# paulmillr/noble-curves

Hardware: NVIDIA H100
Metric: BLS12-381 G1 MSM points/sec at 2^20 scalars (higher is better)
Workload: dtype u32-limb integer (381-bit Fp, Montgomery)

## Files before the change

noble-curves_b200/csrc/capi.cu:

```cuda
#include <dlfcn.h>
#include <thread>
#include <nccl.h>

#include "context.h"
#include "curve_consts.cuh"
#include "field.cuh"

namespace nmsm {

Context g_ctx;
std::mutex g_mu;
DistState g_dist;

struct NcclApi {
  void* handle = nullptr;
  ncclResult_t (*GetUniqueId)(ncclUniqueId*) = nullptr;
  ncclResult_t (*CommInitRank)(ncclComm_t*, int, ncclUniqueId, int) = nullptr;
  ncclResult_t (*CommDestroy)(ncclComm_t) = nullptr;
  ncclResult_t (*Send)(const void*, size_t, ncclDataType_t, int, ncclComm_t, cudaStream_t) = nullptr;
  ncclResult_t (*Recv)(void*, size_t, ncclDataType_t, int, ncclComm_t, cudaStream_t) = nullptr;
  ncclResult_t (*AllGather)(const void*, void*, size_t, ncclDataType_t, ncclComm_t, cudaStream_t) = nullptr;
  ncclResult_t (*GroupStart)() = nullptr;
  ncclResult_t (*GroupEnd)() = nullptr;
  const char* (*GetErrorString)(ncclResult_t) = nullptr;
// ... 222 lines not shown
  CK(cudaMemcpyAsync(d_h + D.world, &mine, sizeof(mine), cudaMemcpyHostToDevice, st));
  if (int r = nccl_all_gather(d_h + D.world, d_h, sizeof(mine), st)) { cudaFree(d_h); return r; }
  std::vector<cudaIpcMemHandle_t> all(D.world);
  CK(cudaMemcpyAsync(all.data(), d_h, sizeof(mine) * D.world, cudaMemcpyDeviceToHost, st));
  CK(cudaStreamSynchronize(st));
  cudaFree(d_h);
  uint32_t ok = 1;
  for (int r = 0; r < D.world; r++) {
    if (r == D.rank) continue;
    cudaError_t e = cudaIpcOpenMemHandle(&D.mapped[slot][r], all[r], cudaIpcMemLazyEnablePeerAccess);
    if (e != cudaSuccess) {
      (void)cudaGetLastError();
      D.mapped[slot][r] = nullptr;
      ok = 0;
    }
  }
  uint32_t* d_ok = nullptr;
  CK(cudaMalloc((void**)&d_ok, 4 * (D.world + 1)));
  CK(cudaMemcpyAsync(d_ok + D.world, &ok, 4, cudaMemcpyHostToDevice, st));
  if (int r = nccl_all_gather(d_ok + D.world, d_ok, 4, st)) { cudaFree(d_ok); return r; }
  std::vector<uint32_t> oks(D.world);
  CK(cudaMemcpyAsync(oks.data(), d_ok, 4 * D.world, cudaMemcpyDeviceToHost, st));
  CK(cudaStreamSynchronize(st));
  cudaFree(d_ok);
  for (uint32_t v : oks) ok &= v;
  if (!ok) {
    for (int r = 0; r < D.world; r++)
      if (D.mapped[slot][r]) {
        cudaIpcCloseMemHandle(D.mapped[slot][r]);
        D.mapped[slot][r] = nullptr;
      }
    D.p2p = false;
    return NMSM_OK;
  }
  D.mapped_local[slot] = local_base;
  return NMSM_OK;
}

}

using namespace nmsm;

#define ENGINE(curve)                                      \
  const EngineVTable* E = engine_for(curve);               \
  if (!E) return fail(NMSM_ERR_ARG, "unknown curve id")
#define SLOT0_FREE()                                                                                         \
  if (g_ctx.slot[0].pend.active)                                                                             \
  return fail(NMSM_ERR_ARG, "slot 0 holds an MSM that has not been collected: collect it before a synchronous call")

extern "C" {

int nmsm_init(int device) {
  std::lock_guard<std::mutex> lk(g_mu);
  Context& C = g_ctx;
  if (C.ready && C.device == device) return NMSM_OK;
  if (C.ready) return fail(NMSM_ERR_ARG, "nmsm_init: context already bound to another device");
  setenv("CUDA_DEVICE_MAX_CONNECTIONS", "32", 0);
  int count = 0;
  cudaError_t e = cudaGetDeviceCount(&count);
  if (e != cudaSuccess || count == 0)
    return fail(NMSM_ERR_CUDA, std::string("no CUDA device available (there is no CPU fallback): ") +
                                   cudaGetErrorString(e));
  if (device < 0 || device >= count) return fail(NMSM_ERR_ARG, "nmsm_init: bad device ordinal");
  CK(cudaSetDevice(device));
  cudaDeviceProp prop;
  CK(cudaGetDeviceProperties(&prop, device));
  C.sm_count = prop.multiProcessorCount;
  int prio_lo = 0, prio_hi = 0;
  CK(cudaDeviceGetStreamPriorityRange(&prio_lo, &prio_hi));
  for (Slot& S : C.slot) {
    CK(cudaStreamCreateWithFlags(&S.stream, cudaStreamNonBlocking));
    for (auto& st : S.acc_stream) CK(cudaStreamCreateWithPriority(&st, cudaStreamNonBlocking, prio_lo));
    for (auto& st : S.tail_stream) CK(cudaStreamCreateWithPriority(&st, cudaStreamNonBlocking, prio_hi));
    CK(cudaStreamCreateWithPriority(&S.horner_stream, cudaStreamNonBlocking, prio_hi));
    CK(cudaStreamCreateWithFlags(&S.prep_stream, cudaStreamNonBlocking));
    CK(cudaEventCreateWithFlags(&S.ev_start, cudaEventDisableTiming));
    CK(cudaEventCreateWithFlags(&S.ev_prep, cudaEventDisableTiming));
    CK(cudaMallocHost((void**)&S.h_result, 1024));
    for (auto& ev : S.ev) CK(cudaEventCreate(&ev));
    CK(cudaEventCreateWithFlags(&S.done, cudaEventDisableTiming));
    CK(cudaEventCreateWithFlags(&S.ev_fork, cudaEventDisableTiming));
    CK(cudaEventCreateWithFlags(&S.ev_horner, cudaEventDisableTiming));
    for (auto& ev : S.ev_acc) CK(cudaEventCreateWithFlags(&ev, cudaEventDisableTiming));
    for (auto& ev : S.ev_tail) CK(cudaEventCreateWithFlags(&ev, cudaEventDisableTiming));
    CK(cudaEventCreate(&S.ev_t0));
    CK(cudaEventCreate(&S.ev_t1));
    if (getenv("NMSM_TRACE")) {
      C.trace = true;
      CK(cudaEventCreate(&S.tr_fork));
      for (auto& ev : S.tr_acc) CK(cudaEventCreate(&ev));
      for (auto& ev : S.tr_tail) CK(cudaEventCreate(&ev));
      for (auto& ev : S.tr_h) CK(cudaEventCreate(&ev));
    }
    CK(cudaStreamCreateWithPriority(&S.comm_stream, cudaStreamNonBlocking, prio_hi));
    CK(cudaEventCreateWithFlags(&S.ev_gather, cudaEventDisableTiming));
    for (auto& ev : S.ev_fin) CK(cudaEventCreateWithFlags(&ev, cudaEventDisableTiming));
    for (auto& ev : S.ev_xchg) CK(cudaEventCreateWithFlags(&ev, cudaEventDisableTiming));
    CK(cudaMallocHost((void**)&S.h_gather, 64 * 1024));
  }
  C.device = device;
  C.ready = true;
  return NMSM_OK;
}

void nmsm_shutdown(void) {
  std::lock_guard<std::mutex> lk(g_mu);
  Context& C = g_ctx;
  if (!C.ready) return;
  if (g_dist.ready) {
    for (Slot& S : C.slot) cudaStreamSynchronize(S.comm_stream);
    for (int sl = 0; sl < NUM_SLOTS; sl++)
      for (int r = 0; r < MAX_PEERS; r++)
        if (g_dist.mapped[sl][r]) cudaIpcCloseMemHandle(g_dist.mapped[sl][r]);
    g_nccl.CommDestroy((ncclComm_t)g_dist.comm);
    g_dist = DistState();
  }
  for (Slot& S : C.slot) {
    cudaStreamSynchronize(S.stream);
    cudaStreamSynchronize(S.comm_stream);
    for (auto st : S.acc_stream) cudaStreamSynchronize(st);
    for (auto st : S.tail_stream) cudaStreamSynchronize(st);
    cudaStreamSynchronize(S.horner_stream);
    cudaStreamSynchronize(S.prep_stream);
    for (Buf* b : {&S.in_pts, &S.in_scalars, &S.aff, &S.counts, &S.offsets, &S.cursor, &S.sorted, &S.buckets, &S.heads,
                   &S.tails, &S.chunk_out, &S.window_out, &S.tile_sums, &S.blk, &S.tiles, &S.result, &S.mul_out, &S.hacc,
                   &S.recv, &S.gsend, &S.grecv})
      b->release();
    for (auto& ev : S.ev_fin) cudaEventDestroy(ev);
    for (auto& ev : S.ev_xchg) cudaEventDestroy(ev);
    cudaEventDestroy(S.ev_gather);
    cudaFreeHost(S.h_gather);
    cudaStreamDestroy(S.comm_stream);
    for (auto& ev : S.ev) cudaEventDestroy(ev);
    for (auto& ev : S.ev_acc) cudaEventDestroy(ev);
    for (auto& ev : S.ev_tail) cudaEventDestroy(ev);
    for (cudaEvent_t ev : {S.done, S.ev_fork, S.ev_horner, S.ev_t0, S.ev_t1}) cudaEventDestroy(ev);
    cudaFreeHost(S.h_result);
    for (auto st : S.acc_stream) cudaStreamDestroy(st);
    for (auto st : S.tail_stream) cudaStreamDestroy(st);
    cudaStreamDestroy(S.horner_stream);
    cudaStreamDestroy(S.prep_stream);
    cudaEventDestroy(S.ev_start);
    cudaEventDestroy(S.ev_prep);
    cudaStreamDestroy(S.stream);
    S.pend = Pending();
  }
  h2d_release();
  C.ed_scratch.release();
  cudaFree(C.secp256k1_g_table);
  C.secp256k1_g_table = nullptr;
  cudaFree(C.p256_g_table);
  C.p256_g_table = nullptr;
  cudaFree(C.ed25519_b_table);
  C.ed25519_b_table = nullptr;
  for (Buf* b : {&C.ntt_data, &C.ntt_work, &C.ntt_tmp, &C.ntt_roots, &C.ntt_aux}) b->release();
  C.ntt_key_field = -1;
  C.ntt_key_bits = -1;
  C.ready = false;
  C.device = -1;
}

const char* nmsm_last_error(void) {
  static thread_local std::string copy;
  std::lock_guard<std::mutex> lk(g_mu);
  copy = g_ctx.last_error;
  return copy.c_str();
}
long long nmsm_last_error_index(void) {
  std::lock_guard<std::mutex> lk(g_mu);
  return g_ctx.last_error_index;
}

int nmsm_point_bytes(int curve) {
  ENGINE(curve);
  return E->point_bytes;
}
int nmsm_acc_bytes(int curve) {
  ENGINE(curve);
  return E->acc_bytes;
}

int nmsm_msm(int curve, const uint8_t* pts, const uint8_t* scalars, uint64_t n, uint8_t* out_xy, int* out_is_inf) {
  std::lock_guard<std::mutex> lk(g_mu);
  if (int r = ensure_init()) return r;
  g_ctx.cur = 0;
  SLOT0_FREE();
  if (!out_xy || !out_is_inf || (n && (!pts || !scalars))) return fail(NMSM_ERR_ARG, "null pointer");
  ENGINE(curve);
  return E->msm_host(pts, scalars, n, out_xy, out_is_inf);
}

int nmsm_msm_device(int curve, const void* d_pts, const void* d_scalars, uint64_t n, uint8_t* out_xy,
                    int* out_is_inf) {
  std::lock_guard<std::mutex> lk(g_mu);
  if (int r = ensure_init()) return r;
  g_ctx.cur = 0;
  SLOT0_FREE();
  if (!out_xy || !out_is_inf || (n && (!d_pts || !d_scalars))) return fail(NMSM_ERR_ARG, "null pointer");
  ENGINE(curve);
  return E->msm_device((const uint32_t*)d_pts, (const uint32_t*)d_scalars, n, nullptr, out_xy, out_is_inf);
}

int nmsm_msm_partial_device(int curve, const void* d_pts, const void* d_scalars, uint64_t n, void* d_out_acc) {
  std::lock_guard<std::mutex> lk(g_mu);
  if (int r = ensure_init()) return r;
  g_ctx.cur = 0;
  SLOT0_FREE();
  if (!d_out_acc || (n && (!d_pts || !d_scalars))) return fail(NMSM_ERR_ARG, "null pointer");
  ENGINE(curve);
  return E->msm_device((const uint32_t*)d_pts, (const uint32_t*)d_scalars, n, (uint32_t*)d_out_acc, nullptr, nullptr);
}

int nmsm_fold_partials_device(int curve, const void* d_accs, int count, uint8_t* out_xy, int* out_is_inf) {
  std::lock_guard<std::mutex> lk(g_mu);
  if (int r = ensure_init()) return r;
  g_ctx.cur = 0;
  SLOT0_FREE();
// ... 521 lines not shown
```

noble-curves_b200/csrc/context.h:

```cpp
#pragma once
#include <cuda_runtime.h>
#include <stdint.h>
#include <stdio.h>
#include <string.h>

#include <mutex>
#include <string>
#include <vector>

#include "../../include/nmsm.h"

namespace nmsm {
struct MsmPlanLite {
  int c, W, B, G, L, K, chunks, D;
  uint32_t TPW;
};
}

namespace nmsm {

struct Buf {
  void* p = nullptr;
  size_t cap = 0;
  cudaError_t ensure(size_t bytes) {
    if (bytes <= cap) return cudaSuccess;
    if (p) cudaFree(p);
    p = nullptr;
    cap = 0;
    size_t want = bytes + bytes / 8 + 256;
    cudaError_t e = cudaMalloc(&p, want);
    if (e == cudaSuccess) cap = want;
    return e;
  }
  void release() {
    if (p) cudaFree(p);
    p = nullptr;
    cap = 0;
  }
};

struct Pending {
  bool active = false;
  int curve = -1;
  MsmPlanLite plan = {};
  uint64_t n = 0;
  bool partial = false;
  bool empty = false;
  bool sharded = false;
  int gather_words = 0;
  bool profiled = false;
  int groups = 1;
  int launches = 0;
};
static constexpr int MAX_GROUPS = 8;
static constexpr int MAX_WINDOWS = 34;
static constexpr int ACC_STREAMS = 8, TAIL_STREAMS = 4;
struct Slot {
  cudaStream_t stream = nullptr;
  cudaStream_t acc_stream[ACC_STREAMS] = {}, tail_stream[TAIL_STREAMS] = {}, horner_stream = nullptr;
  cudaStream_t prep_stream = nullptr;
  cudaEvent_t ev_start = nullptr, ev_prep = nullptr;
  cudaEvent_t ev_fork = nullptr, ev_acc[MAX_WINDOWS] = {}, ev_tail[MAX_WINDOWS] = {}, ev_horner = nullptr;
  cudaStream_t comm_stream = nullptr;
  cudaEvent_t ev_fin[MAX_WINDOWS] = {}, ev_xchg[MAX_WINDOWS] = {}, ev_gather = nullptr;
  uint32_t* h_gather = nullptr;
  Buf recv, gsend, grecv;
  cudaEvent_t ev_t0 = nullptr, ev_t1 = nullptr;
  cudaEvent_t tr_fork = nullptr, tr_acc[MAX_WINDOWS] = {}, tr_tail[MAX_WINDOWS] = {}, tr_h[MAX_WINDOWS] = {};
  Buf in_pts, in_scalars, aff, counts, offsets, cursor, sorted, buckets, heads, tails, chunk_out, window_out, tile_sums,
      blk, tiles, result, mul_out, hacc;
  uint32_t* h_result = nullptr;
  cudaEvent_t ev[NMSM_TIMING_SLOTS + 2] = {};
  cudaEvent_t done = nullptr;
  float last_ms[NMSM_TIMING_SLOTS] = {};
  nmsm_plan_info last_info = {};
  Pending pend;
};
static constexpr int NUM_SLOTS = NMSM_SLOTS;

struct Context {
  bool ready = false;
  int device = -1;
  int sm_count = 132;
  Slot slot[NUM_SLOTS];
  int cur = 0;
  Buf ed_scratch;
  uint32_t* secp256k1_g_table = nullptr;
  uint32_t* ed25519_b_table = nullptr;
  uint32_t* p256_g_table = nullptr;
  Buf ntt_data, ntt_work, ntt_tmp, ntt_roots, ntt_aux;
  int ntt_key_field = -1, ntt_key_bits = -1;
  uint64_t ntt_key_gen = 0;
  bool profiling = false;
  bool trace = false;
  int forced_c = 0;
  int forced_groups = 0;
  float last_ms[NMSM_TIMING_SLOTS] = {};
  nmsm_plan_info last_info = {};
  std::string last_error;
  long long last_error_index = -1;
};

int h2d_any(void* dst, const void* src, size_t bytes, cudaStream_t stream);
void h2d_release();

struct NcclComm;
static constexpr int MAX_PEERS = 16;
struct PeerPtrs {
  const uint32_t* p[MAX_PEERS];
};
struct DistState {
  bool ready = false;
  int rank = 0, world = 1;
  NcclComm* comm = nullptr;
  bool p2p = false;
  void* mapped[NMSM_SLOTS][MAX_PEERS] = {};
  void* mapped_local[NMSM_SLOTS] = {};
};
int nccl_send(const void* buf, size_t bytes, int peer, cudaStream_t st);
int nccl_recv(void* buf, size_t bytes, int peer, cudaStream_t st);
int nccl_group_start();
int nccl_group_end();
int nccl_all_gather(const void* send, void* recv, size_t bytes_per_rank, cudaStream_t st);
int dist_map_peer_buckets(int slot, void* local_base, cudaStream_t st);
extern DistState g_dist;

struct ShardArgs {
  uint64_t n_total, offset;
};

extern Context g_ctx;
extern std::mutex g_mu;

inline int fail(int code, const std::string& msg, long long idx = -1) {
  g_ctx.last_error = msg;
  g_ctx.last_error_index = idx;
  return code;
}
inline int cuda_fail(cudaError_t e, const char* what) {
  return fail(NMSM_ERR_CUDA, std::string("CUDA error in ") + what + ": " + cudaGetErrorString(e));
}
#define CK(call)                                         \
  do {                                                   \
    cudaError_t e__ = (call);                            \
    if (e__ != cudaSuccess) return cuda_fail(e__, #call); \
  } while (0)

inline int check_offsets(const uint64_t* off, const char* name, uint64_t n) {
  if (off[0] != 0) return fail(NMSM_ERR_ARG, std::string(name) + "[0] must be 0");
  for (uint64_t i = 0; i < n; i++)
    if (off[i + 1] < off[i])
      return fail(NMSM_ERR_ARG, std::string(name) + " must be non-decreasing (index " + std::to_string(i + 1) + ")",
// ... 85 lines not shown
```

noble-curves_b200/csrc/engine.cuh:

```cuda
#pragma once
#include "context.h"
#include "msm.cuh"

namespace nmsm {

inline unsigned int cdiv(uint64_t a, unsigned int b) { return (unsigned int)((a + b - 1) / b); }

#define EV(slot)                                                         \
  do {                                                                   \
    if (g_ctx.profiling) cudaEventRecord(C.ev[slot], C.stream);              \
  } while (0)

template <class Cv>
struct Engine {
  using G = typename Cv::G;

static int run_msm(const uint32_t* d_pts, const uint32_t* d_scalars, uint64_t n, uint32_t* d_out_acc,
                   uint8_t* out_xy, int* out_is_inf, const uint32_t* d_prepared = nullptr, int table_c = 0,
                   uint64_t table_points = 0) {
  if (int r = submit_msm(d_pts, d_scalars, n, d_out_acc, d_prepared, table_c, table_points)) return r;
  return collect_msm(out_xy, out_is_inf);
}

static int reduce2_r(uint64_t chunks) {
  if (chunks <= (uint64_t)REDUCE2_LOGICAL * 4) {
    int r = 1;
    while ((uint64_t)REDUCE2_LOGICAL * r < chunks) r *= 2;
    return r;
  }
  int r = REDUCE2_R;
  while (r < 16 && (chunks + (uint64_t)REDUCE2_LOGICAL * r - 1) / ((uint64_t)REDUCE2_LOGICAL * r) > (uint64_t)REDUCE2_MAX_SPLITS &&
         chunks <= (uint64_t)REDUCE2_LOGICAL * 16 * REDUCE2_MAX_SPLITS)
    r *= 2;
  return r;
}

static constexpr int SHARD_MIN_C = 8;

static int choose_groups(const MsmPlan& plan, uint64_t max_entries) {
  (void)max_entries;
  if (plan.W <= 1) return 1;
  int ng = 1;
  if (g_ctx.forced_groups) ng = g_ctx.forced_groups < plan.W ? g_ctx.forced_groups : plan.W;
  if (g_ctx.profiling) ng = 1;
  return ng;
}

static bool prepare_on_side_stream(uint64_t n, bool prepared) { return !g_ctx.profiling && !prepared && n >= (1u << 14); }

static int stage_host_inputs(Slot& C, const void* pts, const void* scalars, uint64_t n) {
  if (n >= (1ull << 31)) return fail(NMSM_ERR_ARG, "n must be < 2^31");
  CK(C.in_pts.ensure(n * G::IN_WORDS * 4));
  CK(C.in_scalars.ensure(n * SCALAR_WORDS * 4));
  if (int r = h2d_any(C.in_scalars.p, scalars, n * SCALAR_WORDS * 4, C.stream)) return r;
  return h2d_any(C.in_pts.p, pts, n * G::IN_WORDS * 4, prepare_on_side_stream(n, false) ? C.prep_stream : C.stream);
}

static int submit_msm(const uint32_t* d_pts, const uint32_t* d_scalars, uint64_t n, uint32_t* d_out_acc,
                      const uint32_t* d_prepared, int table_c = 0, uint64_t table_points = 0,
                      const ShardArgs* shard = nullptr) {
  Slot& C = g_ctx.slot[g_ctx.cur];
  if (C.pend.active) return fail(NMSM_ERR_ARG, "slot busy: collect the previous MSM first");
  if (n >= (1ull << 31)) return fail(NMSM_ERR_ARG, "n must be < 2^31");
  if (shard && (!g_dist.ready || d_out_acc || d_prepared))
    return fail(NMSM_ERR_ARG, shard && !g_dist.ready ? "nmsm_dist_init has not been called" : "sharded MSM: unsupported combination");
  const uint64_t n_plan = shard ? shard->n_total : n;
  if (shard && (n_plan >= (1ull << 31) || shard->offset + n > n_plan)) return fail(NMSM_ERR_ARG, "sharded MSM: bad shard bounds");
  const int RES_WORDS = G::IN_WORDS + 4;
  CK(C.result.ensure((RES_WORDS + 4) * 4));
  uint32_t* d_res = (uint32_t*)C.result.p;
  unsigned int* d_err = (unsigned int*)(d_res + G::IN_WORDS + 1);

  C.pend = Pending();
  C.pend.curve = Cv::ID;
  C.pend.n = n;
  C.pend.partial = d_out_acc != nullptr;
  if (n_plan == 0) {
    if (d_out_acc) {
      typename G::Acc id = G::identity();
      CK(cudaMemcpyAsync(d_out_acc, &id, sizeof(id), cudaMemcpyHostToDevice, C.stream));
      CK(cudaStreamSynchronize(C.stream));
    }
    C.pend.empty = true;
    C.pend.active = true;
    return NMSM_OK;
  }

  MsmPlan plan = table_c ? make_table_plan<Cv>(table_points, table_c, g_ctx.sm_count)
                         : make_plan<Cv>(n_plan, g_ctx.forced_c, g_ctx.sm_count, shard ? (n ? n : 1) : 0, shard ? SHARD_MIN_C : 2);
  if (shard && plan.W > MAX_WINDOWS) return fail(NMSM_ERR_ARG, "window count exceeds MAX_WINDOWS");
  if (shard && g_ctx.forced_groups > 1) plan_one_wave_per_window<Cv>(plan, n, g_ctx.sm_count);
  const uint64_t max_entries = (n ? n : 1) * (uint64_t)plan.D * split_of<Cv>();
  if (max_entries >= (1ull << 32)) return fail(NMSM_ERR_ARG, "n * windows must be < 2^32");
  size_t blk_entries = 0;
  for (uint64_t m = plan.chunks;;) {
    const uint64_t sp = (m + (uint64_t)REDUCE2_LOGICAL * reduce2_r(m) - 1) / ((uint64_t)REDUCE2_LOGICAL * reduce2_r(m));
    blk_entries += sp;
    if (sp <= 1) break;
    m = sp;
  }
  const uint64_t nseg = (uint64_t)plan.W * plan.TPW;

  if (!d_prepared) CK(C.aff.ensure((n ? n : 1) * split_of<Cv>() * G::AFF_WORDS * 4));
  CK(C.counts.ensure((size_t)(plan.G + 1) * 4));
  CK(C.offsets.ensure((size_t)(plan.G + 1) * 4));
  CK(C.cursor.ensure((size_t)(plan.G + 1) * 4));
  CK(C.sorted.ensure(max_entries * 4));
  CK(C.buckets.ensure((size_t)plan.G * G::ACC_WORDS * 4));
  CK(C.heads.ensure(nseg * G::ACC_WORDS * 4));
  CK(C.tails.ensure(nseg * G::ACC_WORDS * 4));
  CK(C.chunk_out.ensure((size_t)plan.W * plan.chunks * G::ACC_WORDS * 4 * 2));
  CK(C.tile_sums.ensure((size_t)(plan.G / SCAN_TILE + 2) * 4));
  const uint64_t ntile1 = nseg / STITCH_FAN, ntile2 = ntile1 / STITCH_FAN;
  CK(C.tiles.ensure((ntile1 + ntile2) * G::ACC_WORDS * 4));
  CK(C.blk.ensure((size_t)plan.W * blk_entries * G::ACC_WORDS * 4 * 2));
  CK(C.window_out.ensure((size_t)plan.W * G::ACC_WORDS * 4));
  CK(C.hacc.ensure((size_t)G::ACC_WORDS * 4));

  uint32_t* aff = d_prepared ? const_cast<uint32_t*>(d_prepared) : (uint32_t*)C.aff.p;
  unsigned int* counts = (unsigned int*)C.counts.p;
  uint32_t* offsets = (uint32_t*)C.offsets.p;
  unsigned int* cursor = (unsigned int*)C.cursor.p;
  uint32_t* sorted = (uint32_t*)C.sorted.p;
  uint32_t* buckets = (uint32_t*)C.buckets.p;
  uint32_t* heads = (uint32_t*)C.heads.p;
  uint32_t* tails = (uint32_t*)C.tails.p;
  uint32_t* sums = (uint32_t*)C.chunk_out.p;
  uint32_t* wsums = sums + (size_t)plan.W * plan.chunks * G::ACC_WORDS;
  uint32_t* tile_sums = (uint32_t*)C.tile_sums.p;
  uint32_t* tile1 = (uint32_t*)C.tiles.p;
  uint32_t* tile2 = tile1 + ntile1 * G::ACC_WORDS;
  uint32_t* window_out = (uint32_t*)C.window_out.p;
  uint32_t* hacc = (uint32_t*)C.hacc.p;
  cudaStream_t st = C.stream;
  const uint32_t n32 = (uint32_t)n;
  int NG = choose_groups(plan, max_entries);
  if (shard) {
    NG = g_ctx.forced_groups ? (g_ctx.forced_groups >= plan.W ? plan.W : g_ctx.forced_groups) : 1;
    if (NG > 1) NG = plan.W;
  }
  static const int quad_env = getenv("NMSM_QUAD_REDUCE1") ? atoi(getenv("NMSM_QUAD_REDUCE1")) : 0;
  const bool quad_reduce1 = (quad_env == 1 && NG > 1) || quad_env == 2 || (quad_env == 0 && NG == 1 && reduce1_quad_form(plan));
  const bool prof = g_ctx.profiling && !shard;
  const int world = shard ? g_dist.world : 1, rank = shard ? g_dist.rank : 0;
  const int slots = (plan.W + world - 1) / world;
  const size_t WB = (size_t)plan.B * G::ACC_WORDS;
  const int gather_words = slots * G::ACC_WORDS + 4;
  uint32_t *recv = nullptr, *gsend = nullptr, *grecv = nullptr;
  bool p2p = shard && g_dist.p2p && world > 1;
  PeerPtrs peer_ptrs = {};
  if (shard) {
    if (p2p) {
      if (int r = dist_map_peer_buckets(g_ctx.cur, C.buckets.p, C.comm_stream)) return r;
      p2p = g_dist.p2p;
      for (int r = 0; r < world && p2p; r++) peer_ptrs.p[r] = (const uint32_t*)g_dist.mapped[g_ctx.cur][r];
    }
    if (!p2p) CK(C.recv.ensure((size_t)slots * (world - 1) * WB * 4 + 16));
    CK(C.gsend.ensure((size_t)gather_words * 4));
    CK(C.grecv.ensure((size_t)gather_words * 4 * world + 256 + 4 * world));
    recv = (uint32_t*)C.recv.p;
    gsend = (uint32_t*)C.gsend.p;
    grecv = (uint32_t*)C.grecv.p;
  }
  int launches = 0;
#define PEV(slot)                                   \
  do {                                              \
    if (prof) cudaEventRecord(C.ev[slot], st);      \
  } while (0)

  CK(cudaEventRecord(C.ev_t0, st));
  PEV(0);
  CK(cudaMemsetAsync(d_err, 0xff, 8, st));
  CK(cudaMemsetAsync(counts, 0, (size_t)(plan.G + 1) * 4, st));
  const bool prep_aside = prepare_on_side_stream(n, d_prepared != nullptr);
  if (!d_prepared && n) {
    cudaStream_t sp = prep_aside ? C.prep_stream : st;
    if (prep_aside) {
      CK(cudaEventRecord(C.ev_start, st));
      CK(cudaStreamWaitEvent(sp, C.ev_start, 0));
    }
    k_prepare<Cv><<<cdiv(n, 128), 128, 0, sp>>>(d_pts, n32, aff, d_err);
    if (prep_aside) CK(cudaEventRecord(C.ev_prep, sp));
    launches++;
  }
  PEV(1);
  if (n) k_digits<Cv, false><<<cdiv(n, 256), 256, 0, st>>>(d_scalars, n32, plan, counts, nullptr, d_err);
  PEV(2);
  {
    const unsigned int tiles = cdiv(plan.G, SCAN_TILE);
    k_scan_tiles<<<tiles, SCAN_THREADS, 0, st>>>(counts, (uint32_t)plan.G, tile_sums);
    k_scan_apply<<<tiles, SCAN_THREADS, 0, st>>>(counts, (uint32_t)plan.G, tile_sums, offsets, cursor);
  }
  PEV(3);
  if (n) k_digits<Cv, true><<<cdiv(n, 256), 256, 0, st>>>(d_scalars, n32, plan, cursor, sorted, d_err);
  launches += 4;
  PEV(4);
  if (prof) {
    CK(cudaMemsetAsync(d_res + RES_WORDS, 0, 16, st));
    const uint64_t items = nseg > (uint64_t)plan.G ? nseg : (uint64_t)plan.G;
    k_count_starts<<<cdiv(items, 256), 256, 0, st>>>(offsets, plan, (unsigned long long*)(d_res + RES_WORDS));
    cudaEventRecord(C.ev[4], st);
  }
  if (shard) { k_set_identity<Cv><<<1, 32, 0, st>>>(gsend, slots); launches++; }
  if (prep_aside) CK(cudaStreamWaitEvent(st, C.ev_prep, 0));
  if (NG > 1) CK(cudaEventRecord(C.ev_fork, st));
  const bool trace = g_ctx.trace && (NG > 1 || shard);
  if (trace) cudaEventRecord(C.tr_fork, st);

  const int per = (plan.W + NG - 1) / NG;
  int ngroups = 0;
  for (int w_hi = plan.W; w_hi > 0; w_hi -= per, ngroups++) {
    const int w_lo = w_hi > per ? w_hi - per : 0;
    const uint32_t nw = (uint32_t)(w_hi - w_lo);
    cudaStream_t sa = NG > 1 ? C.acc_stream[ngroups % ACC_STREAMS] : st;
    if (NG > 1 && ngroups < ACC_STREAMS) CK(cudaStreamWaitEvent(sa, C.ev_fork, 0));
    k_accumulate<Cv><<<cdiv((uint64_t)nw * plan.TPW, 128), 128, 0, sa>>>(aff, sorted, offsets, plan, (uint32_t)w_lo, buckets,
                                                                         heads, tails);
    if (NG > 1) CK(cudaEventRecord(C.ev_acc[ngroups], sa));
    if (trace) cudaEventRecord(C.tr_acc[ngroups], sa);
  }
  if (shard) {
    const size_t smem2 = (REDUCE2_THREADS / 32) * G::ACC_WORDS * 4;
    int g = 0;
    for (int w_hi = plan.W; w_hi > 0; w_hi -= per, g++) {
      const int w_lo = w_hi > per ? w_hi - per : 0;
      cudaStream_t stl = NG > 1 ? C.tail_stream[g % TAIL_STREAMS] : st;
      if (NG > 1) CK(cudaStreamWaitEvent(stl, C.ev_acc[g], 0));
      {
        const uint32_t a0 = (uint32_t)((uint64_t)w_lo * plan.TPW / STITCH_FAN), a1 = (uint32_t)((uint64_t)w_hi * plan.TPW / STITCH_FAN);
        k_stitch_tiles<Cv><<<cdiv((uint64_t)(a1 - a0) * 32, 128), 128, 0, stl>>>(offsets, plan, STITCH_FAN, a0, a1, heads, tile1);
        const uint32_t b0 = a0 / STITCH_FAN, b1 = a1 / STITCH_FAN;
        k_stitch_tiles<Cv><<<cdiv((uint64_t)(b1 - b0) * 32, 128), 128, 0, stl>>>(offsets, plan, STITCH_FAN * STITCH_FAN, b0, b1,
                                                                                tile1, tile2);
        k_bucket_finalize<Cv><<<cdiv((uint64_t)(w_hi - w_lo) * plan.B, 128), 128, 0, stl>>>(
            offsets, buckets, heads, tails, tile1, tile2, plan, (uint32_t)w_lo * plan.B, (uint32_t)w_hi * plan.B);
        launches += 3;
      }
      if (world > 1 && p2p) {
        CK(cudaEventRecord(C.ev_fin[g], stl));
        CK(cudaStreamWaitEvent(C.comm_stream, C.ev_fin[g], 0));
        if (nccl_all_gather(grecv + (size_t)gather_words * world + 16, grecv + (size_t)gather_words * world + 32, 4, C.comm_stream))
          return NMSM_ERR_CUDA;
        CK(cudaEventRecord(C.ev_xchg[g], C.comm_stream));
        if (trace) cudaEventRecord(C.tr_h[g], C.comm_stream);
      } else if (world > 1) {
        CK(cudaEventRecord(C.ev_fin[g], stl));
        CK(cudaStreamWaitEvent(C.comm_stream, C.ev_fin[g], 0));
        if (nccl_group_start()) return NMSM_ERR_CUDA;
        for (int w = w_hi - 1; w >= w_lo; w--) {
          const int own_rank = w % world;
          if (own_rank == rank) {
            uint32_t* wrecv = recv + (size_t)(w / world) * (world - 1) * WB;
            for (int r = 0, k = 0; r < world; r++)
              if (r != rank && nccl_recv(wrecv + (size_t)(k++) * WB, WB * 4, r, C.comm_stream)) return NMSM_ERR_CUDA;
          } else if (nccl_send(buckets + (size_t)w * WB, WB * 4, own_rank, C.comm_stream)) {
            return NMSM_ERR_CUDA;
          }
        }
        if (nccl_group_end()) return NMSM_ERR_CUDA;
        CK(cudaEventRecord(C.ev_xchg[g], C.comm_stream));
        if (trace) cudaEventRecord(C.tr_h[g], C.comm_stream);
      } else {
        CK(cudaEventRecord(C.ev_xchg[g], stl));
      }
      if (trace) cudaEventRecord(C.tr_tail[g], stl);
      for (int w = w_hi - 1; w >= w_lo; w--) {
        if (w % world != rank) continue;
        const int slot = w / world;
        cudaStream_t so = C.tail_stream[slot % TAIL_STREAMS];
        CK(cudaStreamWaitEvent(so, C.ev_xchg[g], 0));
        uint32_t* wb = buckets + (size_t)w * WB;
        if (world > 1 && p2p) {
          k_bucket_fold_peers<Cv><<<cdiv((uint64_t)plan.B * 4, 128), 128, 0, so>>>(wb, peer_ptrs, (size_t)w * WB, world, rank,
                                                                                (uint32_t)plan.B);
          launches++;
        } else if (world > 1) {
          k_bucket_fold<Cv><<<cdiv((uint64_t)plan.B * 4, 128), 128, 0, so>>>(wb, recv + (size_t)slot * (world - 1) * WB, world - 1, WB,
                                                                          (uint32_t)plan.B);
          launches++;
        }
        const uint32_t id0 = (uint32_t)w * plan.chunks, id1 = id0 + plan.chunks;
        k_reduce1_dense<Cv><<<cdiv((uint64_t)(id1 - id0) * 4, REDUCE1_THREADS), REDUCE1_THREADS, 0, so>>>(buckets, plan, id0, id1, sums,
                                                                                                    wsums);
        launches++;
        MsmPlan pl = plan;
        const uint32_t *S = sums, *T = wsums;
        uint32_t* base = (uint32_t*)C.blk.p;
        for (;;) {
          const int R2 = reduce2_r(pl.chunks), per_block = REDUCE2_LOGICAL * R2;
          const int splits = (pl.chunks + per_block - 1) / per_block;
          uint32_t* blkP = base;
          uint32_t* blkQ = base + (size_t)plan.W * splits * G::ACC_WORDS;
          base = blkQ + (size_t)plan.W * splits * G::ACC_WORDS;
          k_reduce2<Cv><<<dim3(splits, 1), REDUCE2_THREADS, smem2, so>>>(S, T, pl, R2, (uint32_t)w, blkP, blkQ,
// ... 510 lines not shown
```

noble-curves_b200/csrc/msm.cuh:

```cuda
#pragma once
#include <cuda_runtime.h>
#include <stdint.h>

#include "msm_body.cuh"
#include "validate.cuh"

namespace nmsm {

template <class Cv>
__global__ void k_prepare(const uint32_t* __restrict__ pts, uint32_t n, uint32_t* __restrict__ aff,
                          unsigned int* err) {
  uint32_t i = blockIdx.x * blockDim.x + threadIdx.x;
  if (i < n) prepare_body<Cv>(i, n, pts, aff, err);
}

template <class Cv, bool SCATTER>
__global__ void k_digits(const uint32_t* __restrict__ scalars, uint32_t n, MsmPlan plan,
                         unsigned int* __restrict__ counts_or_cursor, uint32_t* __restrict__ sorted,
                         unsigned int* err) {
  uint32_t i = blockIdx.x * blockDim.x + threadIdx.x;
  if (i < n) digits_body<Cv, SCATTER>(i, n, scalars, plan, counts_or_cursor, sorted, err);
}

static constexpr int SCAN_THREADS = 256;
static constexpr int SCAN_PER_THREAD = 8;
static constexpr int SCAN_TILE = SCAN_THREADS * SCAN_PER_THREAD;

__device__ __forceinline__ uint32_t block_sum_256(uint32_t v, uint32_t* sh) {
  for (int d = 16; d >= 1; d >>= 1) v += __shfl_down_sync(0xffffffffu, v, d);
  if ((threadIdx.x & 31) == 0) sh[threadIdx.x >> 5] = v;
  __syncthreads();
  uint32_t t = 0;
  for (int q = 0; q < SCAN_THREADS / 32; q++) t += sh[q];
  __syncthreads();
  return t;
}

static __global__ void __launch_bounds__(SCAN_THREADS)
k_scan_tiles(const unsigned int* __restrict__ counts, uint32_t G, uint32_t* __restrict__ tile_sums) {
  __shared__ uint32_t sh[SCAN_THREADS / 32];
  const uint32_t base = blockIdx.x * SCAN_TILE + threadIdx.x * SCAN_PER_THREAD;
  uint32_t v = 0;
#pragma unroll
  for (int k = 0; k < SCAN_PER_THREAD; k++)
    if (base + k < G) v += counts[base + k];
  uint32_t t = block_sum_256(v, sh);
  if (threadIdx.x == 0) tile_sums[blockIdx.x] = t;
}

static __global__ void __launch_bounds__(SCAN_THREADS)
k_scan_apply(const unsigned int* __restrict__ counts, uint32_t G, const uint32_t* __restrict__ tile_sums,
             uint32_t* __restrict__ offsets, unsigned int* __restrict__ cursor) {
  __shared__ uint32_t sh[SCAN_THREADS / 32];
  __shared__ uint32_t warp_tot[SCAN_THREADS / 32];
  uint32_t pre = 0;
  for (uint32_t k = threadIdx.x; k < blockIdx.x; k += SCAN_THREADS) pre += tile_sums[k];
  const uint32_t tile_prefix = block_sum_256(pre, sh);
  const uint32_t base = blockIdx.x * SCAN_TILE + threadIdx.x * SCAN_PER_THREAD;
  uint32_t c[SCAN_PER_THREAD];
  uint32_t mine = 0;
#pragma unroll
  for (int k = 0; k < SCAN_PER_THREAD; k++) {
    c[k] = (base + k < G) ? counts[base + k] : 0;
    mine += c[k];
  }
  const uint32_t lane = threadIdx.x & 31, warp = threadIdx.x >> 5;
  uint32_t inc = mine;
  for (int d = 1; d < 32; d <<= 1) {
    uint32_t o = __shfl_up_sync(0xffffffffu, inc, d);
    if (lane >= (uint32_t)d) inc += o;
  }
  if (lane == 31) warp_tot[warp] = inc;
  __syncthreads();
  uint32_t wpre = 0;
  for (uint32_t q = 0; q < warp; q++) wpre += warp_tot[q];
  uint32_t run = tile_prefix + wpre + inc - mine;
#pragma unroll
  for (int k = 0; k < SCAN_PER_THREAD; k++) {
    if (base + k < G) {
      offsets[base + k] = run;
      cursor[base + k] = run;
    }
    run += c[k];
  }
  if (base < G && base + SCAN_PER_THREAD >= G) offsets[G] = run;
}

template <class F>
__device__ __forceinline__ F shfl_field(const F& a, int src_lane) {
  F r;
  const uint32_t* s = reinterpret_cast<const uint32_t*>(&a);
  uint32_t* d = reinterpret_cast<uint32_t*>(&r);
#pragma unroll
  for (int k = 0; k < (int)(sizeof(F) / 4); k++) d[k] = __shfl_sync(0xffffffffu, s[k], src_lane);
  return r;
}
template <class F>
__device__ __noinline__ F warp_batch_inverse(const F& z) {
  const int lane = threadIdx.x & 31;
  F pre = z, suf = z;
  for (int d = 1; d < 32; d <<= 1) {
    F a = shfl_field(pre, lane >= d ? lane - d : lane);
    F b = shfl_field(suf, lane + d < 32 ? lane + d : lane);
    if (lane >= d) pre = pre * a;
// ... 391 lines not shown
```

noble-curves_b200/csrc/msm_body.cuh:

```cuda
#pragma once
#include <math.h>
#include <stdint.h>
#include <stdlib.h>

#include "ec.cuh"

#if defined(__CUDACC__)
#define NMSM_NL __host__ __device__ __noinline__
#else
#define NMSM_NL inline
#endif

namespace nmsm {

static constexpr int MAX_WINDOW_BITS = 16;
static constexpr int MAX_TABLE_BITS = 22;
static constexpr int SCALAR_WORDS = 8;

struct MsmPlan {
  int c;
  int W;
  int B;
  int G;
  int L;
// ... 591 lines not shown
    }
    const F2 cx{a.x.c0, -a.x.c1}, cy{a.y.c0, -a.y.c1};
    typename G::Affine t;
    t.x = cx * px;
    t.y = cy * py;
    store_words<G::AFF_WORDS>(aff + (size_t)(n + i) * G::AFF_WORDS, reinterpret_cast<const uint32_t*>(&t));
    t.x = F2{a.x.c0 * p2x, a.x.c1 * p2x};
    t.y = -a.y;
    store_words<G::AFF_WORDS>(aff + (size_t)(2 * (size_t)n + i) * G::AFF_WORDS, reinterpret_cast<const uint32_t*>(&t));
    t.x = cx * p3x;
    t.y = cy * p3y;
    store_words<G::AFF_WORDS>(aff + (size_t)(3 * (size_t)n + i) * G::AFF_WORDS, reinterpret_cast<const uint32_t*>(&t));
  } else if constexpr (Cv::GLV) {
    typename G::Field beta;
    for (int k = 0; k < G::Field::LIMBS; k++) beta.v[k] = Cv::Glv::BETA_MONT(k);
    a.x = a.x * beta;
    store_words<G::AFF_WORDS>(aff + (size_t)(n + i) * G::AFF_WORDS, reinterpret_cast<const uint32_t*>(&a));
  }
}

template <class Cv>
NMSM_HD void table_level_body(uint32_t i, const uint32_t* prev, uint32_t* next, int c) {
  using G = typename Cv::G;
  typename G::Affine a = load_aff<G>(prev + (size_t)i * G::AFF_WORDS);
  typename G::Acc acc = G::from_affine(a);
  for (int j = 0; j < c; j++) nl_dbl<G>(acc);
  a = G::to_affine_prepared(acc);
  store_words<G::AFF_WORDS>(next + (size_t)i * G::AFF_WORDS, reinterpret_cast<const uint32_t*>(&a));
}

static constexpr int PT_BITS = 16;
static constexpr uint32_t PT_HALF = 1u << (PT_BITS - 1);
template <class Cv, int BITS = PT_BITS>
NMSM_HD constexpr int point_table_levels() { return (Cv::Fn::BITS + 1 + BITS - 1) / BITS; }

template <class Cv, int BITS = PT_BITS>
NMSM_HD void table_base_body(uint32_t i, const uint32_t* p_aff, uint32_t* level0) {
  using G = typename Cv::G;
  const typename G::Affine P = load_aff<G>(p_aff);
  typename G::Acc acc = G::identity();
  const uint32_t k = i + 1;
  for (int b = BITS - 1; b >= 0; b--) {
    nl_dbl<G>(acc);
    if ((k >> b) & 1u) nl_madd<G>(acc, P);
  }
  typename G::Affine a = G::to_affine_prepared(acc);
  store_words<G::AFF_WORDS>(level0 + (size_t)i * G::AFF_WORDS, reinterpret_cast<const uint32_t*>(&a));
}

template <class Cv, int BITS = PT_BITS>
NMSM_HD bool table_mul_body(uint32_t i, const uint32_t* tbl, const uint32_t* scalars, int allow_zero,
                            typename Cv::G::Acc& acc, unsigned int* err) {
  using G = typename Cv::G;
  constexpr uint32_t HALF = 1u << (BITS - 1);
  uint32_t s[SCALAR_WORDS];
  load_words<SCALAR_WORDS>(s, scalars + (size_t)i * SCALAR_WORDS);
  uint32_t nz = 0;
  for (int k = 0; k < SCALAR_WORDS; k++) nz |= s[k];
  acc = G::identity();
  if (!scalar_in_range<typename Cv::Fn>(s) || (!allow_zero && nz == 0)) {
    atomic_min_u32(&err[1], i);
    return false;
  }
  uint32_t carry = 0;
  constexpr int LEVELS = point_table_levels<Cv, BITS>();
  for (int w = 0; w < LEVELS; w++) {
    uint32_t v = scalar_bits(s, w * BITS, BITS) + carry;
    carry = 0;
    bool neg = false;
    if (v > HALF) {
      v = (1u << BITS) - v;
      neg = true;
      carry = 1;
    }
    if (v != 0) {
      typename G::Affine a = load_aff<G>(tbl + ((size_t)w * HALF + (v - 1)) * G::AFF_WORDS);
      a = G::cneg(a, neg);
      nl_madd<G>(acc, a);
    }
  }
  return true;
}

template <bool SCATTER>
NMSM_HD void emit_digits(const uint32_t* m, int nwords, uint32_t index, uint32_t flip, const MsmPlan& plan,
                         unsigned int* counts_or_cursor, uint32_t* sorted) {
  uint32_t carry = 0;
  for (int w = 0; w < plan.D; w++) {
    const int width = digit_width(plan, w);
    const uint32_t half = 1u << (width - 1);
    uint32_t v = scalar_bits(m, digit_offset(plan, w), width, nwords) + carry;
    carry = 0;
    uint32_t neg = flip;
    if (v > half) {
      v = (1u << width) - v;
      neg ^= 1u;
      carry = 1;
    }
    if (v != 0) {
      const uint32_t g = (plan.stride ? 0u : (uint32_t)w * (uint32_t)plan.B) + (v - 1);
      if (SCATTER) {
        uint32_t pos = atomic_add_u32(&counts_or_cursor[g], 1u);
        sorted[pos] = (index + (uint32_t)w * plan.stride) | (neg << 31);
      } else {
        atomic_add_u32(&counts_or_cursor[g], 1u);
      }
    }
  }
}

template <class Cv, bool SCATTER>
NMSM_HD void digits_body(uint32_t i, uint32_t n, const uint32_t* scalars, const MsmPlan& plan,
                         unsigned int* counts_or_cursor, uint32_t* sorted, unsigned int* err) {
  uint32_t s[SCALAR_WORDS];
  load_words<SCALAR_WORDS>(s, scalars + (size_t)i * SCALAR_WORDS);
  if (!scalar_in_range<typename Cv::Fn>(s)) {
    if (!SCATTER) atomic_min_u32(&err[1], i);
    return;
  }
  if constexpr (Cv::GLV_KIND == 1) {
    uint32_t m1[4], m2[4];
    bool neg1, neg2;
    glv_split<typename Cv::Glv>(s, m1, neg1, m2, neg2);
    emit_digits<SCATTER>(m1, 4, i, neg1 ? 1u : 0u, plan, counts_or_cursor, sorted);
    emit_digits<SCATTER>(m2, 4, n + i, neg2 ? 1u : 0u, plan, counts_or_cursor, sorted);
  } else if constexpr (Cv::GLV_KIND == 2) {
    uint32_t m1[5], m2[5];
    bool neg1, neg2;
    glv_split_lattice<typename Cv::Glv>(s, m1, neg1, m2, neg2);
    emit_digits<SCATTER>(m1, 5, i, neg1 ? 1u : 0u, plan, counts_or_cursor, sorted);
    emit_digits<SCATTER>(m2, 5, n + i, neg2 ? 1u : 0u, plan, counts_or_cursor, sorted);
  } else if constexpr (Cv::GLV_KIND == 3) {
    uint64_t mag[4];
    bool neg[4];
    gls_split<typename Cv::Glv>(s, mag, neg);
    for (int j = 0; j < 4; j++) {
      const uint32_t m[2] = {(uint32_t)mag[j], (uint32_t)(mag[j] >> 32)};
      emit_digits<SCATTER>(m, 2, (uint32_t)j * n + i, (neg[j] ? 1u : 0u) ^ (uint32_t)(j & 1), plan, counts_or_cursor, sorted);
    }
  } else {
    emit_digits<SCATTER>(s, SCALAR_WORDS, i, 0u, plan, counts_or_cursor, sorted);
  }
}

template <class Cv>
NMSM_HD void accumulate_body(uint32_t w, uint32_t t, const uint32_t* aff, const uint32_t* sorted, const uint32_t* offsets,
                             const MsmPlan& plan, uint32_t* buckets, uint32_t* heads, uint32_t* tails) {
  using G = typename Cv::G;
  const uint32_t g_lo = w * (uint32_t)plan.B, g_hi = g_lo + (uint32_t)plan.B;
  const uint32_t base = offsets[g_lo], T = offsets[g_hi];
  const uint64_t seg64 = (uint64_t)base + (uint64_t)t * (uint32_t)plan.L;
  if (seg64 >= T) return;
  const uint32_t seg = (uint32_t)seg64;
  const uint32_t end = (T - seg > (uint32_t)plan.L) ? seg + plan.L : T;
  const size_t sid = (size_t)w * plan.TPW + t;
  uint32_t lo = g_lo, hi = g_hi;
  while (hi - lo > 1) {
    uint32_t mid = (lo + hi) >> 1;
    if (offsets[mid] <= seg) lo = mid; else hi = mid;
  }
  uint32_t g = lo;
  uint32_t bstart = offsets[g], bend = offsets[g + 1];
  typename G::Acc acc = G::identity();
  auto next_bucket = [&](uint32_t pos) {
    if (bstart >= seg) save_acc<G>(buckets + (size_t)g * G::ACC_WORDS, acc);
    else save_acc<G>(heads + sid * G::ACC_WORDS, acc);
    acc = G::identity();
    do { g++; } while (offsets[g + 1] <= pos);
    bstart = offsets[g];
    bend = offsets[g + 1];
  };
#if defined(__CUDA_ARCH__)
  if constexpr (acc_inline_products<G>()) {
    constexpr int Q = G::AFF_WORDS / 4;
    __shared__ uint4 next_pts[2][Q][128];
    uint32_t e = sorted[seg], e_next = seg + 1 < end ? sorted[seg + 1] : 0u;
    load_words_async<G::AFF_WORDS>(next_pts[0], aff + (size_t)(e & 0x7fffffffu) * G::AFF_WORDS);
    for (uint32_t pos = seg, slot = 0; pos < end; pos++, slot ^= 1u) {
      if (pos == bend) next_bucket(pos);
      const uint32_t e_after = pos + 2 < end ? sorted[pos + 2] : 0u;
      if (pos + 1 < end) load_words_async<G::AFF_WORDS>(next_pts[slot ^ 1u], aff + (size_t)(e_next & 0x7fffffffu) * G::AFF_WORDS);
      else asm volatile("cp.async.commit_group;" ::: "memory");
      asm volatile("cp.async.wait_group 1;" ::: "memory");
      typename G::Affine a;
      uint32_t* aw = reinterpret_cast<uint32_t*>(&a);
#pragma unroll
      for (int k = 0; k < Q; k++) {
        const uint4 v = next_pts[slot][k][threadIdx.x];
        aw[4 * k] = v.x;
        aw[4 * k + 1] = v.y;
        aw[4 * k + 2] = v.z;
        aw[4 * k + 3] = v.w;
      }
      a = G::cneg(a, (e >> 31) != 0);
      G::template madd<true>(acc, a);
      e = e_next;
      e_next = e_after;
    }
  } else
#endif
  {
    for (uint32_t pos = seg; pos < end; pos++) {
      if (pos == bend) next_bucket(pos);
      uint32_t e = sorted[pos];
      typename G::Affine a = load_aff<G>(aff + (size_t)(e & 0x7fffffffu) * G::AFF_WORDS);
      a = G::cneg(a, (e >> 31) != 0);
      if constexpr (acc_inline_products<G>()) G::template madd<true>(acc, a);
      else G::madd(acc, a);
    }
  }
  const bool head_open = bstart < seg;
  const bool tail_open = bend > end;
  if (!head_open && !tail_open) save_acc<G>(buckets + (size_t)g * G::ACC_WORDS, acc);
  else if (head_open) save_acc<G>(heads + sid * G::ACC_WORDS, acc);
  else save_acc<G>(tails + sid * G::ACC_WORDS, acc);
}

static constexpr int MAX_PAIRS = 32;

template <class F>
NMSM_HD bool pair_usable(const F& x1, const F& x2) {
  return !x1.is_zero() && !x2.is_zero() && x1 != x2;
}

template <class Cv>
// ... 474 lines not shown
```

Before: 109.4 million.

## Recode scalars once, scatter per window, and overlap accumulation with scatter

Scalar recoding (GLV split and signed digits) now runs once and stores per-window digit entries to a new buffer, so the second full recode pass that existed only to scatter is gone. Scatter is then launched one window at a time from the highest window down. When there is a single group and no sharding, each window's bucket accumulation starts on a round-robin accumulation stream as soon as its scatter finishes, overlapping sorting with accumulation. This costs an extra digits buffer of one word per term per window, more kernel launches and more event traffic, and the per-window scatter kernels reread the digit array with streaming loads.

```diff
diff --git a/noble-curves_b200/csrc/capi.cu b/noble-curves_b200/csrc/capi.cu
--- a/noble-curves_b200/csrc/capi.cu
+++ b/noble-curves_b200/csrc/capi.cu
@@ -328,6 +328,7 @@
     CK(cudaEventCreateWithFlags(&S.ev_fork, cudaEventDisableTiming));
     CK(cudaEventCreateWithFlags(&S.ev_horner, cudaEventDisableTiming));
     for (auto& ev : S.ev_acc) CK(cudaEventCreateWithFlags(&ev, cudaEventDisableTiming));
+    CK(cudaEventCreateWithFlags(&S.ev_scat, cudaEventDisableTiming));
     for (auto& ev : S.ev_tail) CK(cudaEventCreateWithFlags(&ev, cudaEventDisableTiming));
     CK(cudaEventCreate(&S.ev_t0));
     CK(cudaEventCreate(&S.ev_t1));
@@ -368,7 +369,7 @@
     for (auto st : S.tail_stream) cudaStreamSynchronize(st);
     cudaStreamSynchronize(S.horner_stream);
     cudaStreamSynchronize(S.prep_stream);
-    for (Buf* b : {&S.in_pts, &S.in_scalars, &S.aff, &S.counts, &S.offsets, &S.cursor, &S.sorted, &S.buckets, &S.heads,
+    for (Buf* b : {&S.in_pts, &S.in_scalars, &S.aff, &S.counts, &S.digits, &S.offsets, &S.cursor, &S.sorted, &S.buckets, &S.heads,
                    &S.tails, &S.chunk_out, &S.window_out, &S.tile_sums, &S.blk, &S.tiles, &S.result, &S.mul_out, &S.hacc,
                    &S.recv, &S.gsend, &S.grecv})
       b->release();
@@ -379,6 +380,7 @@
     cudaStreamDestroy(S.comm_stream);
     for (auto& ev : S.ev) cudaEventDestroy(ev);
     for (auto& ev : S.ev_acc) cudaEventDestroy(ev);
+    cudaEventDestroy(S.ev_scat);
     for (auto& ev : S.ev_tail) cudaEventDestroy(ev);
     for (cudaEvent_t ev : {S.done, S.ev_fork, S.ev_horner, S.ev_t0, S.ev_t1}) cudaEventDestroy(ev);
     cudaFreeHost(S.h_result);
diff --git a/noble-curves_b200/csrc/context.h b/noble-curves_b200/csrc/context.h
--- a/noble-curves_b200/csrc/context.h
+++ b/noble-curves_b200/csrc/context.h
@@ -61,13 +61,14 @@
   cudaStream_t prep_stream = nullptr;
   cudaEvent_t ev_start = nullptr, ev_prep = nullptr;
   cudaEvent_t ev_fork = nullptr, ev_acc[MAX_WINDOWS] = {}, ev_tail[MAX_WINDOWS] = {}, ev_horner = nullptr;
+  cudaEvent_t ev_scat = nullptr;
   cudaStream_t comm_stream = nullptr;
   cudaEvent_t ev_fin[MAX_WINDOWS] = {}, ev_xchg[MAX_WINDOWS] = {}, ev_gather = nullptr;
   uint32_t* h_gather = nullptr;
   Buf recv, gsend, grecv;
   cudaEvent_t ev_t0 = nullptr, ev_t1 = nullptr;
   cudaEvent_t tr_fork = nullptr, tr_acc[MAX_WINDOWS] = {}, tr_tail[MAX_WINDOWS] = {}, tr_h[MAX_WINDOWS] = {};
-  Buf in_pts, in_scalars, aff, counts, offsets, cursor, sorted, buckets, heads, tails, chunk_out, window_out, tile_sums,
+  Buf in_pts, in_scalars, aff, counts, digits, offsets, cursor, sorted, buckets, heads, tails, chunk_out, window_out, tile_sums,
       blk, tiles, result, mul_out, hacc;
   uint32_t* h_result = nullptr;
   cudaEvent_t ev[NMSM_TIMING_SLOTS + 2] = {};
diff --git a/noble-curves_b200/csrc/engine.cuh b/noble-curves_b200/csrc/engine.cuh
--- a/noble-curves_b200/csrc/engine.cuh
+++ b/noble-curves_b200/csrc/engine.cuh
@@ -105,6 +105,7 @@
   CK(C.counts.ensure((size_t)(plan.G + 1) * 4));
   CK(C.offsets.ensure((size_t)(plan.G + 1) * 4));
   CK(C.cursor.ensure((size_t)(plan.G + 1) * 4));
+  CK(C.digits.ensure(max_entries * 4));
   CK(C.sorted.ensure(max_entries * 4));
   CK(C.buckets.ensure((size_t)plan.G * G::ACC_WORDS * 4));
   CK(C.heads.ensure(nseg * G::ACC_WORDS * 4));
@@ -119,6 +120,7 @@
 
   uint32_t* aff = d_prepared ? const_cast<uint32_t*>(d_prepared) : (uint32_t*)C.aff.p;
   unsigned int* counts = (unsigned int*)C.counts.p;
+  uint32_t* digits = (uint32_t*)C.digits.p;
   uint32_t* offsets = (uint32_t*)C.offsets.p;
   unsigned int* cursor = (unsigned int*)C.cursor.p;
   uint32_t* sorted = (uint32_t*)C.sorted.p;
@@ -184,16 +186,32 @@
     launches++;
   }
   PEV(1);
-  if (n) k_digits<Cv, false><<<cdiv(n, 256), 256, 0, st>>>(d_scalars, n32, plan, counts, nullptr, d_err);
+  if (n) k_recode<Cv><<<cdiv(n, 256), 256, 0, st>>>(d_scalars, n32, plan, counts, digits, d_err);
   PEV(2);
   {
     const unsigned int tiles = cdiv(plan.G, SCAN_TILE);
     k_scan_tiles<<<tiles, SCAN_THREADS, 0, st>>>(counts, (uint32_t)plan.G, tile_sums);
     k_scan_apply<<<tiles, SCAN_THREADS, 0, st>>>(counts, (uint32_t)plan.G, tile_sums, offsets, cursor);
   }
+  launches += 3;
   PEV(3);
-  if (n) k_digits<Cv, true><<<cdiv(n, 256), 256, 0, st>>>(d_scalars, n32, plan, cursor, sorted, d_err);
-  launches += 4;
+  const bool acc_per_window = !shard && !prof && NG == 1 && plan.W > 1 && plan.stride == 0 && n;
+  const uint64_t terms = n * (uint64_t)split_of<Cv>();
+  for (int d = plan.D - 1; d >= 0 && n; d--) {
+    k_scatter<<<cdiv(terms, 256), 256, 0, st>>>(digits, terms, d, plan, cursor, sorted);
+    launches++;
+    if (acc_per_window) {
+      const int sx = d % ACC_STREAMS;
+      CK(cudaEventRecord(C.ev_scat, st));
+      CK(cudaStreamWaitEvent(C.acc_stream[sx], C.ev_scat, 0));
+      if (prep_aside) CK(cudaStreamWaitEvent(C.acc_stream[sx], C.ev_prep, 0));
+      k_accumulate<Cv><<<cdiv(plan.TPW, 128), 128, 0, C.acc_stream[sx]>>>(aff, sorted, offsets, plan, (uint32_t)d, buckets,
+                                                                          heads, tails);
+      CK(cudaEventRecord(C.ev_acc[sx], C.acc_stream[sx]));
+    }
+  }
+  if (acc_per_window)
+    for (int sx = 0; sx < ACC_STREAMS && sx < plan.W; sx++) CK(cudaStreamWaitEvent(st, C.ev_acc[sx], 0));
   PEV(4);
   if (prof) {
     CK(cudaMemsetAsync(d_res + RES_WORDS, 0, 16, st));
@@ -210,6 +228,7 @@
   const int per = (plan.W + NG - 1) / NG;
   int ngroups = 0;
   for (int w_hi = plan.W; w_hi > 0; w_hi -= per, ngroups++) {
+    if (acc_per_window) continue;
     const int w_lo = w_hi > per ? w_hi - per : 0;
     const uint32_t nw = (uint32_t)(w_hi - w_lo);
     cudaStream_t sa = NG > 1 ? C.acc_stream[ngroups % ACC_STREAMS] : st;
diff --git a/noble-curves_b200/csrc/msm.cuh b/noble-curves_b200/csrc/msm.cuh
--- a/noble-curves_b200/csrc/msm.cuh
+++ b/noble-curves_b200/csrc/msm.cuh
@@ -14,12 +14,17 @@
   if (i < n) prepare_body<Cv>(i, n, pts, aff, err);
 }
 
-template <class Cv, bool SCATTER>
-__global__ void k_digits(const uint32_t* __restrict__ scalars, uint32_t n, MsmPlan plan,
-                         unsigned int* __restrict__ counts_or_cursor, uint32_t* __restrict__ sorted,
-                         unsigned int* err) {
+template <class Cv>
+__global__ void k_recode(const uint32_t* __restrict__ scalars, uint32_t n, MsmPlan plan, unsigned int* __restrict__ counts,
+                         uint32_t* __restrict__ digits, unsigned int* err) {
   uint32_t i = blockIdx.x * blockDim.x + threadIdx.x;
-  if (i < n) digits_body<Cv, SCATTER>(i, n, scalars, plan, counts_or_cursor, sorted, err);
+  if (i < n) recode_body<Cv>(i, n, scalars, plan, counts, digits, err);
+}
+
+static __global__ void k_scatter(const uint32_t* __restrict__ digits, uint64_t terms, int d, MsmPlan plan,
+                                 unsigned int* __restrict__ cursor, uint32_t* __restrict__ sorted) {
+  const uint64_t j = (uint64_t)blockIdx.x * blockDim.x + threadIdx.x;
+  if (j < terms) scatter_body((uint32_t)j, terms, d, plan, digits, cursor, sorted);
 }
 
 static constexpr int SCAN_THREADS = 256;
diff --git a/noble-curves_b200/csrc/msm_body.cuh b/noble-curves_b200/csrc/msm_body.cuh
--- a/noble-curves_b200/csrc/msm_body.cuh
+++ b/noble-curves_b200/csrc/msm_body.cuh
@@ -697,9 +697,9 @@
   return true;
 }
 
-template <bool SCATTER>
-NMSM_HD void emit_digits(const uint32_t* m, int nwords, uint32_t index, uint32_t flip, const MsmPlan& plan,
-                         unsigned int* counts_or_cursor, uint32_t* sorted) {
+static constexpr uint32_t NO_DIGIT = 0xffffffffu;
+template <class Sink>
+NMSM_HD void recode_digits(const uint32_t* m, int nwords, uint32_t j, uint32_t flip, const MsmPlan& plan, Sink& sink) {
   uint32_t carry = 0;
   for (int w = 0; w < plan.D; w++) {
     const int width = digit_width(plan, w);
@@ -712,50 +712,98 @@
       neg ^= 1u;
       carry = 1;
     }
-    if (v != 0) {
-      const uint32_t g = (plan.stride ? 0u : (uint32_t)w * (uint32_t)plan.B) + (v - 1);
-      if (SCATTER) {
-        uint32_t pos = atomic_add_u32(&counts_or_cursor[g], 1u);
-        sorted[pos] = (index + (uint32_t)w * plan.stride) | (neg << 31);
-      } else {
-        atomic_add_u32(&counts_or_cursor[g], 1u);
-      }
-    }
-  }
-}
-
-template <class Cv, bool SCATTER>
-NMSM_HD void digits_body(uint32_t i, uint32_t n, const uint32_t* scalars, const MsmPlan& plan,
-                         unsigned int* counts_or_cursor, uint32_t* sorted, unsigned int* err) {
+    uint32_t e = NO_DIGIT;
+    if (v != 0) e = ((plan.stride ? 0u : (uint32_t)w * (uint32_t)plan.B) + (v - 1)) | (neg << 31);
+    sink(j, w, e);
+  }
+}
+
+template <class Cv, class Sink>
+NMSM_HD void recode_scalar(uint32_t i, uint32_t n, const uint32_t* scalars, const MsmPlan& plan, unsigned int* err, Sink& sink) {
   uint32_t s[SCALAR_WORDS];
   load_words<SCALAR_WORDS>(s, scalars + (size_t)i * SCALAR_WORDS);
   if (!scalar_in_range<typename Cv::Fn>(s)) {
-    if (!SCATTER) atomic_min_u32(&err[1], i);
+    atomic_min_u32(&err[1], i);
+    for (int k = 0; k < split_of<Cv>(); k++)
+      for (int w = 0; w < plan.D; w++) sink((uint32_t)k * n + i, w, NO_DIGIT);
     return;
   }
   if constexpr (Cv::GLV_KIND == 1) {
     uint32_t m1[4], m2[4];
     bool neg1, neg2;
     glv_split<typename Cv::Glv>(s, m1, neg1, m2, neg2);
-    emit_digits<SCATTER>(m1, 4, i, neg1 ? 1u : 0u, plan, counts_or_cursor, sorted);
-    emit_digits<SCATTER>(m2, 4, n + i, neg2 ? 1u : 0u, plan, counts_or_cursor, sorted);
+    recode_digits(m1, 4, i, neg1 ? 1u : 0u, plan, sink);
+    recode_digits(m2, 4, n + i, neg2 ? 1u : 0u, plan, sink);
   } else if constexpr (Cv::GLV_KIND == 2) {
     uint32_t m1[5], m2[5];
     bool neg1, neg2;
     glv_split_lattice<typename Cv::Glv>(s, m1, neg1, m2, neg2);
-    emit_digits<SCATTER>(m1, 5, i, neg1 ? 1u : 0u, plan, counts_or_cursor, sorted);
-    emit_digits<SCATTER>(m2, 5, n + i, neg2 ? 1u : 0u, plan, counts_or_cursor, sorted);
+    recode_digits(m1, 5, i, neg1 ? 1u : 0u, plan, sink);
+    recode_digits(m2, 5, n + i, neg2 ? 1u : 0u, plan, sink);
   } else if constexpr (Cv::GLV_KIND == 3) {
     uint64_t mag[4];
     bool neg[4];
     gls_split<typename Cv::Glv>(s, mag, neg);
     for (int j = 0; j < 4; j++) {
       const uint32_t m[2] = {(uint32_t)mag[j], (uint32_t)(mag[j] >> 32)};
-      emit_digits<SCATTER>(m, 2, (uint32_t)j * n + i, (neg[j] ? 1u : 0u) ^ (uint32_t)(j & 1), plan, counts_or_cursor, sorted);
+      recode_digits(m, 2, (uint32_t)j * n + i, (neg[j] ? 1u : 0u) ^ (uint32_t)(j & 1), plan, sink);
     }
   } else {
-    emit_digits<SCATTER>(s, SCALAR_WORDS, i, 0u, plan, counts_or_cursor, sorted);
-  }
+    recode_digits(s, SCALAR_WORDS, i, 0u, plan, sink);
+  }
+}
+
+NMSM_HD void scatter_entry(uint32_t j, int d, uint32_t e, const MsmPlan& plan, unsigned int* cursor, uint32_t* sorted) {
+  const uint32_t pos = atomic_add_u32(&cursor[e & 0x7fffffffu], 1u);
+  sorted[pos] = (j + (uint32_t)d * plan.stride) | (e & 0x80000000u);
+}
+
+struct RecodeSink {
+  unsigned int* counts;
+  uint32_t* digits;
+  uint64_t terms;
+  NMSM_HD void operator()(uint32_t j, int w, uint32_t e) {
+    if (e != NO_DIGIT) atomic_add_u32(&counts[e & 0x7fffffffu], 1u);
+#if defined(__CUDA_ARCH__)
+    __stcs(digits + (size_t)w * terms + j, e);
+#else
+    digits[(size_t)w * terms + j] = e;
+#endif
+  }
+};
+template <class Cv>
+NMSM_HD void recode_body(uint32_t i, uint32_t n, const uint32_t* scalars, const MsmPlan& plan, unsigned int* counts,
+                         uint32_t* digits, unsigned int* err) {
+  RecodeSink sink{counts, digits, (uint64_t)n * split_of<Cv>()};
+  recode_scalar<Cv>(i, n, scalars, plan, err, sink);
+}
+
+NMSM_HD void scatter_body(uint32_t j, uint64_t terms, int d, const MsmPlan& plan, const uint32_t* digits,
+                          unsigned int* cursor, uint32_t* sorted) {
+#if defined(__CUDA_ARCH__)
+  const uint32_t e = __ldcs(digits + (size_t)d * terms + j);
+#else
+  const uint32_t e = digits[(size_t)d * terms + j];
+#endif
+  if (e != NO_DIGIT) scatter_entry(j, d, e, plan, cursor, sorted);
+}
+
+template <bool SCATTER>
+struct ScalarSortSink {
+  unsigned int* counts_or_cursor;
+  uint32_t* sorted;
+  const MsmPlan& plan;
+  NMSM_HD void operator()(uint32_t j, int w, uint32_t e) {
+    if (e == NO_DIGIT) return;
+    if (SCATTER) scatter_entry(j, w, e, plan, counts_or_cursor, sorted);
+    else atomic_add_u32(&counts_or_cursor[e & 0x7fffffffu], 1u);
+  }
+};
+template <class Cv, bool SCATTER>
+NMSM_HD void digits_body(uint32_t i, uint32_t n, const uint32_t* scalars, const MsmPlan& plan,
+                         unsigned int* counts_or_cursor, uint32_t* sorted, unsigned int* err) {
+  ScalarSortSink<SCATTER> sink{counts_or_cursor, sorted, plan};
+  recode_scalar<Cv>(i, n, scalars, plan, err, sink);
 }
 
 template <class Cv>
```

After: 113.8 million, median of 6. 1.04x the previous value.
